# ksahlin/IsoCon

Hardware: AMD Instinct MI355X
Metric: read x candidate alignments/sec (NN-graph build, 50k x 2.5kb reads) (higher is better)
Workload: dtype u64; 1 GPU; C3: 50000 synthetic CCS reads (50000 unique), ~2500 bp, 10 isoforms, seed 30001; 1-set NN graph; edges=78526, graph_digest=65944c838d76a6c9, parallelism=single GPU

## Files before the change

### isocon_amd/csrc/ed_lanes.hpp

```cpp
#pragma once
#include "band_core.hpp"
#include "common.hpp"
#include "ed_lanes_core.hpp"
#include "nn.hpp"

namespace isocon {

template <bool NN>
__global__ __launch_bounds__(256) void k_ed_lanes(DevStore S, NNParams P, const uint32_t *__restrict__ pa, const uint32_t *__restrict__ pb,
                                                   const int32_t *__restrict__ pk, uint64_t n_pairs, int32_t *__restrict__ out)
{
    const uint64_t i = (uint64_t)blockIdx.x * 256u + threadIdx.x;
    uint32_t x = 0, y = 0;
    bool valid = i < n_pairs;
    if (valid) {
        x = pa[i]; y = pb[i];
        valid = x != 0xffffffffu && y != 0xffffffffu && x < S.n && y < S.n && (!NN || x != y);
        if (!valid) { x = 0; y = 0; }
    }
    const int32_t m = S.lens[x], n = S.lens[y];
    bool upd_x = false, upd_y = false;
    int32_t k = -1;
    if (NN) {
        upd_x = valid && P.qflag[x] && P.tflag[y];
        upd_y = valid && P.qflag[y] && P.tflag[x];
        int32_t kx = -1, ky = -1;
        if (upd_x) { const int32_t b = load_relaxed_agent(P.best + x); kx = b < m ? b : m; }
        if (upd_y) { const int32_t b = load_relaxed_agent(P.best + y); ky = b < n ? b : n; }
        k = kx > ky ? kx : ky;
        if (k > 63) k = 63;
    } else if (valid) {
        k = pk[i];
        if (k > 63) k = 63;
    }
    const int32_t d = m - n, ad = d < 0 ? -d : d;
    bool run = valid && k >= 0 && ad <= k;
    int32_t r = -1;
    if (run && (m == 0 || n == 0)) { r = ad; run = false; }
    const uint64_t *planes = S.planes;
    const uint32_t nseq = S.n;
    const int32_t nchunks = (int32_t)S.nchunks;
    auto x_lo = [&](int32_t ci) -> uint64_t { return ci < nchunks ? planes[((size_t)ci * nseq + x) * 2] : 0; };
    auto x_hi = [&](int32_t ci) -> uint64_t { return ci < nchunks ? planes[((size_t)ci * nseq + x) * 2 + 1] : 0; };
    auto y_lo = [&](int32_t ci) -> uint64_t { return ci < nchunks ? planes[((size_t)ci * nseq + y) * 2] : 0; };
    auto y_hi = [&](int32_t ci) -> uint64_t { return ci < nchunks ? planes[((size_t)ci * nseq + y) * 2 + 1] : 0; };
    const int32_t rd = lane_pair_distance(x_lo, x_hi, y_lo, y_hi, m, n, k, run, [](bool b) { return __ballot(b) != 0; });
    if (run) r = rd;
    if (!NN) {
        if (i < n_pairs) out[i] = r;
        return;
    }
    bool hit_x = false, hit_y = false;
    if (r >= P.min_d) {
        if (upd_x && r <= m) hit_x = nn_take(P, x, r);
        if (upd_y && r <= n) hit_y = nn_take(P, y, r);
    }
    nn_append(P, hit_x, (int32_t)x, (int32_t)y, r);
    nn_append(P, hit_y, (int32_t)y, (int32_t)x, r);
}

}
```

### isocon_amd/csrc/ed_lanes_core.hpp

```cpp
#pragma once
#include "band_core.hpp"

namespace isocon {

ISO_HD uint32_t funnel32(uint32_t hi, uint32_t lo, int s)
{
#if defined(__HIP_DEVICE_COMPILE__)
    return __builtin_amdgcn_alignbit(hi, lo, (uint32_t)s);
#else
    return s ? (lo >> s) | (hi << (32 - s)) : lo;
#endif
}

ISO_HD uint32_t splat_bit(uint32_t w, int j)
{
#if defined(__HIP_DEVICE_COMPILE__)
    return (uint32_t)__builtin_amdgcn_sbfe((int)w, (uint32_t)j, 1u);
#else
    return 0u - ((w >> j) & 1u);
#endif
}

ISO_HD uint32_t lane_valid32(int32_t o, int32_t m)
{
    int32_t lo = -o, hi = m - o;
    if (lo < 0) lo = 0;
    if (hi > 32) hi = 32;
    if (hi <= lo) return 0u;
    const uint32_t upto_hi = hi >= 32 ? 0xffffffffu : ((1u << hi) - 1u);
    return upto_hi & ~((1u << lo) - 1u);
}

template <class XL, class XH, class YL, class YH, class Any>
ISO_HD int32_t lane_pair_distance(XL x_lo, XH x_hi, YL y_lo, YH y_hi, int32_t m, int32_t n, int32_t k, bool run, Any any)
{
    const int32_t d = m - n;
    int32_t a0 = lane_emin(d, k < 0 ? 0 : k);
    if (a0 < -63) a0 = -63;
    const int32_t nv = -a0;
    int32_t bstar = d - a0;
    if (bstar < 0) bstar = 0;
    if (bstar > 63) bstar = 63;
    BandLane<1> L;
    band_init<1>(L, nv, bstar);
    int32_t r = -1;
    int32_t o = -nv;
    uint32_t L0, L1, L2, H0, H1, H2;
    {
        const uint64_t tl = ~stream64(x_lo, o), th = ~stream64(x_hi, o);
        L0 = (uint32_t)tl; L1 = (uint32_t)(tl >> 32); H0 = (uint32_t)th; H1 = (uint32_t)(th >> 32);
        L2 = (uint32_t)~stream64(x_lo, o + 64);
        H2 = (uint32_t)~stream64(x_hi, o + 64);
    }
    for (int32_t c0 = 0;; c0 += 32) {
        if (!any(run)) break;
        const uint32_t wl = (uint32_t)stream64(y_lo, c0), wh = (uint32_t)stream64(y_hi, c0);
        const bool full = c0 + 32 <= n;
        if (o >= 0 && !any(run && !full)) {
            uint32_t zreg = 0;
#if defined(__HIP_DEVICE_COMPILE__)
#pragma unroll
#endif
            for (int jj = 0; jj < 32; ++jj) {
                const uint32_t sl = splat_bit(wl, jj), sh = splat_bit(wh, jj);
                const uint32_t nl0 = funnel32(L1, L0, jj), nl1 = funnel32(L2, L1, jj), nh0 = funnel32(H1, H0, jj), nh1 = funnel32(H2, H1, jj);
#if defined(__HIP_DEVICE_COMPILE__)
                const uint32_t e0 = __builtin_amdgcn_bitop3_b32(nl0 ^ sl, nh0, sh, 0x60);
                const uint32_t e1 = __builtin_amdgcn_bitop3_b32(nl1 ^ sl, nh1, sh, 0x60);
#else
                const uint32_t e0 = (nl0 ^ sl) & (nh0 ^ sh), e1 = (nl1 ^ sl) & (nh1 ^ sh);
#endif
                band_step_eq64z(L.VP[0], L.VN[0], zreg, ((uint64_t)e1 << 32) | e0);
            }
#if defined(__HIP_DEVICE_COMPILE__)
            L.ztop += (uint32_t)__popc(zreg);
#else
            L.ztop += (uint32_t)__builtin_popcount(zreg);
#endif
        } else {
            const uint32_t V0 = lane_valid32(o, m), V1 = lane_valid32(o + 32, m), V2 = lane_valid32(o + 64, m);
#if defined(__HIP_DEVICE_COMPILE__)
#pragma unroll 1
#endif
            for (int jj = 0; jj < 32; ++jj) {
                if (run && c0 + jj < n) {
                    uint64_t NL[1], NH[1], VM[1];
                    NL[0] = ((uint64_t)funnel32(L2, L1, jj) << 32) | funnel32(L1, L0, jj);
                    NH[0] = ((uint64_t)funnel32(H2, H1, jj) << 32) | funnel32(H1, H0, jj);
                    VM[0] = ((uint64_t)funnel32(V2, V1, jj) << 32) | funnel32(V1, V0, jj);
                    band_step<1, true>(L, NL, NH, VM, splat_bit(wl, jj), splat_bit(wh, jj));
                }
            }
        }
        if (run) {
            const bool fin = c0 + 32 >= n;
            const int32_t dv = band_diag_value<1>(L, nv, fin ? n : c0 + 32);
            if (fin) { r = dv <= k ? dv : -1; run = false; }
            else if (dv > k) run = false;
        }
        o += 32;
        L0 = L1; L1 = L2; H0 = H1; H1 = H2;
        L2 = (uint32_t)~stream64(x_lo, o + 64);
        H2 = (uint32_t)~stream64(x_hi, o + 64);
    }
    return r;
}

}
```

Before: 72.09 billion alignments/s.

## Prefetch next plane chunks one iteration ahead in lane edit-distance kernel

Restructures the per-lane banded edit-distance loop to step over 64-column words. The next x and y plane chunks are issued as vectorized 128-bit loads before computing two 32-column blocks, with a sched_barrier and asm register pins so the loads stay in flight during compute. It also skips loads beyond the sequence length and replaces the per-iteration stream64 shifting with a precomputed join of 64-bit windows. This adds register pressure and fences that may limit compiler scheduling.

```diff
diff --git a/isocon_amd/csrc/ed_lanes.hpp b/isocon_amd/csrc/ed_lanes.hpp
--- a/isocon_amd/csrc/ed_lanes.hpp
+++ b/isocon_amd/csrc/ed_lanes.hpp
@@ -37,14 +37,20 @@
     bool run = valid && k >= 0 && ad <= k;
     int32_t r = -1;
     if (run && (m == 0 || n == 0)) { r = ad; run = false; }
-    const uint64_t *planes = S.planes;
+    const ulonglong2 *planes = reinterpret_cast<const ulonglong2 *>(S.planes);
     const uint32_t nseq = S.n;
     const int32_t nchunks = (int32_t)S.nchunks;
-    auto x_lo = [&](int32_t ci) -> uint64_t { return ci < nchunks ? planes[((size_t)ci * nseq + x) * 2] : 0; };
-    auto x_hi = [&](int32_t ci) -> uint64_t { return ci < nchunks ? planes[((size_t)ci * nseq + x) * 2 + 1] : 0; };
-    auto y_lo = [&](int32_t ci) -> uint64_t { return ci < nchunks ? planes[((size_t)ci * nseq + y) * 2] : 0; };
-    auto y_hi = [&](int32_t ci) -> uint64_t { return ci < nchunks ? planes[((size_t)ci * nseq + y) * 2 + 1] : 0; };
-    const int32_t rd = lane_pair_distance(x_lo, x_hi, y_lo, y_hi, m, n, k, run, [](bool b) { return __ballot(b) != 0; });
+    auto xp = [&](int32_t ci) -> PlanePair {
+        PlanePair p{0, 0};
+        if (lane_chunk_present(ci, nchunks, m)) { const ulonglong2 v = planes[(size_t)ci * nseq + x]; p.lo = v.x; p.hi = v.y; }
+        return p;
+    };
+    auto yp = [&](int32_t ci) -> PlanePair {
+        PlanePair p{0, 0};
+        if (lane_chunk_present(ci, nchunks, n)) { const ulonglong2 v = planes[(size_t)ci * nseq + y]; p.lo = v.x; p.hi = v.y; }
+        return p;
+    };
+    const int32_t rd = lane_pair_distance_w(xp, yp, m, n, k, run, [](bool b) { return __ballot(b) != 0; });
     if (run) r = rd;
     if (!NN) {
         if (i < n_pairs) out[i] = r;
diff --git a/isocon_amd/csrc/ed_lanes_core.hpp b/isocon_amd/csrc/ed_lanes_core.hpp
--- a/isocon_amd/csrc/ed_lanes_core.hpp
+++ b/isocon_amd/csrc/ed_lanes_core.hpp
@@ -31,8 +31,23 @@
     return upto_hi & ~((1u << lo) - 1u);
 }
 
-template <class XL, class XH, class YL, class YH, class Any>
-ISO_HD int32_t lane_pair_distance(XL x_lo, XH x_hi, YL y_lo, YH y_hi, int32_t m, int32_t n, int32_t k, bool run, Any any)
+struct PlanePair {
+    uint64_t lo, hi;
+};
+
+ISO_HD bool lane_chunk_present(int32_t ci, int32_t nchunks, int32_t len)
+{
+    return ci < nchunks && 64 * ci < len;
+}
+
+#if defined(__HIP_DEVICE_COMPILE__)
+#define ISO_LANES_ARRIVED(p) asm volatile("" : "+v"((p).lo), "+v"((p).hi))
+#else
+#define ISO_LANES_ARRIVED(p) ((void)0)
+#endif
+
+template <class XP, class YP, class Any>
+ISO_HD int32_t lane_pair_distance_w(XP xp, YP yp, int32_t m, int32_t n, int32_t k, bool run, Any any)
 {
     const int32_t d = m - n;
     int32_t a0 = lane_emin(d, k < 0 ? 0 : k);
@@ -44,17 +59,19 @@
     BandLane<1> L;
     band_init<1>(L, nv, bstar);
     int32_t r = -1;
-    int32_t o = -nv;
-    uint32_t L0, L1, L2, H0, H1, H2;
+    auto join = [nv](uint64_t prev, uint64_t next) -> uint64_t { return nv ? (next << nv) | (prev >> (64 - nv)) : next; };
+    uint64_t ul0, ul1, uh0, uh1, cl, ch, yl, yh;
     {
-        const uint64_t tl = ~stream64(x_lo, o), th = ~stream64(x_hi, o);
-        L0 = (uint32_t)tl; L1 = (uint32_t)(tl >> 32); H0 = (uint32_t)th; H1 = (uint32_t)(th >> 32);
-        L2 = (uint32_t)~stream64(x_lo, o + 64);
-        H2 = (uint32_t)~stream64(x_hi, o + 64);
+        PlanePair c0 = xp(0), c1 = xp(1), t0 = yp(0);
+        ISO_LANES_ARRIVED(c0); ISO_LANES_ARRIVED(c1); ISO_LANES_ARRIVED(t0);
+        cl = ~c1.lo; ch = ~c1.hi;
+        ul0 = join(~(uint64_t)0, ~c0.lo); uh0 = join(~(uint64_t)0, ~c0.hi);
+        ul1 = join(~c0.lo, cl); uh1 = join(~c0.hi, ch);
+        yl = t0.lo; yh = t0.hi;
     }
-    for (int32_t c0 = 0;; c0 += 32) {
-        if (!any(run)) break;
-        const uint32_t wl = (uint32_t)stream64(y_lo, c0), wh = (uint32_t)stream64(y_hi, c0);
+    auto block = [&](const int32_t c0, const uint32_t wl, const uint32_t wh, const uint32_t L0, const uint32_t L1, const uint32_t L2,
+                     const uint32_t H0, const uint32_t H1, const uint32_t H2) {
+        const int32_t o = c0 - nv;
         const bool full = c0 + 32 <= n;
         if (o >= 0 && !any(run && !full)) {
             uint32_t zreg = 0;
@@ -98,12 +115,35 @@
             if (fin) { r = dv <= k ? dv : -1; run = false; }
             else if (dv > k) run = false;
         }
-        o += 32;
-        L0 = L1; L1 = L2; H0 = H1; H1 = H2;
-        L2 = (uint32_t)~stream64(x_lo, o + 64);
-        H2 = (uint32_t)~stream64(x_hi, o + 64);
+    };
+    for (int32_t s = 0;; ++s) {
+        if (!any(run)) break;
+        PlanePair tn = yp(s + 1), cn = xp(s + 2);
+#if defined(__HIP_DEVICE_COMPILE__)
+        __builtin_amdgcn_sched_barrier(0);
+#endif
+        block(64 * s, (uint32_t)yl, (uint32_t)yh, (uint32_t)ul0, (uint32_t)(ul0 >> 32), (uint32_t)ul1,
+              (uint32_t)uh0, (uint32_t)(uh0 >> 32), (uint32_t)uh1);
+        if (any(run))
+            block(64 * s + 32, (uint32_t)(yl >> 32), (uint32_t)(yh >> 32), (uint32_t)(ul0 >> 32), (uint32_t)ul1, (uint32_t)(ul1 >> 32),
+                  (uint32_t)(uh0 >> 32), (uint32_t)uh1, (uint32_t)(uh1 >> 32));
+        ISO_LANES_ARRIVED(tn); ISO_LANES_ARRIVED(cn);
+        const uint64_t nl = ~cn.lo, nh = ~cn.hi;
+        ul0 = ul1; uh0 = uh1;
+        ul1 = join(cl, nl); uh1 = join(ch, nh);
+        cl = nl; ch = nh;
+        yl = tn.lo; yh = tn.hi;
     }
     return r;
 }
 
+template <class XL, class XH, class YL, class YH, class Any>
+ISO_HD int32_t lane_pair_distance(XL x_lo, XH x_hi, YL y_lo, YH y_hi, int32_t m, int32_t n, int32_t k, bool run, Any any)
+{
+    return lane_pair_distance_w([&](int32_t ci) -> PlanePair { return PlanePair{x_lo(ci), x_hi(ci)}; },
+                                [&](int32_t ci) -> PlanePair { return PlanePair{y_lo(ci), y_hi(ci)}; }, m, n, k, run, any);
 }
+
+#undef ISO_LANES_ARRIVED
+
+}
```

New measurement: 73.99 billion alignments/s (median of 5 runs). +2.6%, better.
